# Vigilans/GomokuAI

Hardware: AMD Instinct MI355X
Metric: board-evals/s (higher is better)
Workload: dtype int32; 1 GPU; batched AC-automaton position eval (K1), 65536 random-opening boards per GPU, 15x15, inputs resident in HBM; boards_per_gpu=65536, parallelism=boards sharded by rank, no collective, launch=hipGraph replay of the K steps

## Files before the change

gomokuai_amd/csrc/eval_kernel.hip:

```cpp
#include <algorithm>
#include <cstdlib>
#include <vector>

#include "capi_common.h"
#include "host_staging.h"

namespace {

constexpr int kBoardsPerBlock = 16;
constexpr int kGroupBoards = 16;
constexpr int kThreads = 64 * kBoardsPerBlock;
constexpr int kCells = 225;
constexpr int kQueueCap = 448;
constexpr int kMaxBlocksPerCu = 1;
constexpr int kBurstEvery = 12;
static_assert(kBurstEvery >= 1 && kBurstEvery <= kGroupBoards, "every burst of a run needs a board of the run to go with");
[[maybe_unused]] constexpr int kTimelineSlots = 8;

constexpr int kScoreWords = 4 * kCells;
constexpr int kCntWords = 3 * kCells + 1;
constexpr int kZeroWords = kScoreWords + kCntWords;
constexpr int kLineWords = 96;
constexpr int kColBase = 20, kDiagBase = 36, kAntiBase = 65;
#ifndef GMK_K1_TOTALS_COPIES
#define GMK_K1_TOTALS_COPIES 8
#endif
constexpr int kTotalsCopies = GMK_K1_TOTALS_COPIES;
constexpr int kMiscWords = 48;
constexpr int kBoardWords = kZeroWords + kLineWords + kQueueCap + kMiscWords;
static_assert(kZeroWords % 4 == 0 && kBoardWords % 4 == 0, "16-byte alignment of the per-board blocks");
constexpr int kPrefixTableWords = gmk::kPrefixWords;
constexpr int kStaticTableWords = kLineWords + 512 + 1560 + 2 * kPrefixTableWords + 4;

constexpr int kLaneRecordVecs = 2;
constexpr int kSegPads = 2;
constexpr int kScanSteps = 17;
constexpr int kScanPrefixSyms = 4;
constexpr int kPairedLanes = 8, kFirstPairedLane = 64 - kPairedLanes;
constexpr int kSeamStepLong = 8 + kSegPads, kSeamStepShort = 7 + kSegPads;

__device__ __forceinline__ int dir_stride(int dir) { return (0x0E100F01u >> (8 * dir)) & 0xFFu; }

__device__ __forceinline__ uint64_t line_symbols(uint32_t line_word, int len) {
    return static_cast<uint64_t>(line_word) | (0xAull << (2 * len));
}

__device__ __forceinline__ const __attribute__((address_space(3))) uint32_t* lds_word(uint32_t byte_address) {
    return reinterpret_cast<const __attribute__((address_space(3))) uint32_t*>(static_cast<uintptr_t>(byte_address));
}

__device__ __forceinline__ const __attribute__((address_space(3))) uint16_t* lds_half(uint32_t byte_address) {
    return reinterpret_cast<const __attribute__((address_space(3))) uint16_t*>(static_cast<uintptr_t>(byte_address));
}

__device__ __forceinline__ __attribute__((address_space(3))) uint32_t* lds_word_rw(uint32_t byte_address) {
    return reinterpret_cast<__attribute__((address_space(3))) uint32_t*>(static_cast<uintptr_t>(byte_address));
}

__device__ __forceinline__ uint32_t dfa_address(uint32_t table_word, uint32_t four) {
    uint32_t addr;
    asm("v_bfi_b32 %0, %1, %2, %3" : "=v"(addr) : "s"(0x3FF3u), "v"(table_word), "v"(four));
    return addr;
}

__device__ __forceinline__ uint32_t place_advance(uint32_t place, uint32_t lines_word) {
    uint32_t next;
    asm("v_add_u32_sdwa %0, %1, %2 dst_sel:DWORD dst_unused:UNUSED_PAD src0_sel:DWORD src1_sel:BYTE_3" : "=v"(next) : "v"(place), "v"(lines_word));
    return next;
}

template <int kFirstLane>
__device__ __forceinline__ uint32_t place_jump(uint32_t place, int jump) {
    static_assert(kFirstLane >= 0 && kFirstLane < 64 && kFirstLane % 4 == 0, "four lanes of one DPP bank");
    constexpr int kRow = kFirstLane / 16, kBank = (kFirstLane % 16) / 4;
    asm("s_nop 1\n\tv_add_u32_dpp %0, %1, %0 quad_perm:[0,1,2,3] row_mask:%2 bank_mask:%3" : "+v"(place) : "v"(jump), "n"(1 << kRow), "n"(1 << kBank));
    return place;
}

__device__ __forceinline__ uint32_t queue_entry(uint32_t table_word, uint32_t place) {
    uint32_t entry;
    asm("v_bfi_b32 %0, %1, %2, %3" : "=v"(entry) : "s"(0x1FFFFu), "v"(place), "v"(table_word));
    return entry;
}

typedef unsigned short v2u16 __attribute__((ext_vector_type(2)));
__device__ __forceinline__ uint32_t pk_dec_u16(uint32_t word) {
    const v2u16 ones = {1, 1};
    return __builtin_bit_cast(uint32_t, static_cast<v2u16>(__builtin_bit_cast(v2u16, word) - ones));
}

__device__ __forceinline__ void store_saddr(uint32_t byte_offset, int32_t value, unsigned long long base) {
    asm volatile("global_store_dword %0, %1, %2" : : "v"(byte_offset), "v"(value), "s"(base) : "memory");
}

template <int kImm, bool kNt>
__device__ __forceinline__ void store_saddr_imm(uint32_t byte_offset, int32_t value, unsigned long long base) {
    static_assert(kImm >= 0 && kImm < 4096, "the immediate offset of a global store has 13 bits, signed");
    if (kNt) asm volatile("global_store_dword %0, %1, %2 offset:%3 nt" : : "v"(byte_offset), "v"(value), "s"(base), "n"(kImm) : "memory");
    else asm volatile("global_store_dword %0, %1, %2 offset:%3" : : "v"(byte_offset), "v"(value), "s"(base), "n"(kImm) : "memory");
}

__device__ __forceinline__ void wave_phase_fence() {
    __builtin_amdgcn_fence(__ATOMIC_RELEASE, "wavefront");
    __builtin_amdgcn_wave_barrier();
    __builtin_amdgcn_fence(__ATOMIC_ACQUIRE, "wavefront");
}

__device__ __forceinline__ void deposit_match(uint32_t w0, uint32_t w1, int cell_at, int dir, int back_step,
                                              uint32_t* s_scores, uint32_t* s_cnt, uint32_t* s_misc, uint32_t* totals ) {
    const int type = w0 & 15, fav = (w0 >> 4) & 1;
    if (type == 8) { atomicOr(&s_misc[1], fav ? 1u : 2u); return; }
    atomicAdd(&totals[type], fav ? 0x10000u : 1u);
    const int endcell = cell_at + static_cast<int>((w0 >> 27) & 1u) * back_step;
    const uint32_t score = dir >= 2 ? (w1 >> 16) : (w1 & 0xFFFFu);
    unsigned long long* pair = reinterpret_cast<unsigned long long*>(s_scores) + fav;
    const uint32_t lo_opp = fav ? score : 0u, hi_opp = fav ? 0u : score;
    const uint32_t tslot = 5u - static_cast<uint32_t>(type);
    const bool feeds = tslot < 3u;
    uint32_t* cnt = s_cnt + (feeds ? tslot : 0u) * kCells;
    const uint32_t one = 1u << (4 * (fav * 4 + dir));
    const int n_dep = (w0 >> 8) & 7;
#pragma unroll
    for (int d = 0; d < 4; ++d) {
        if (d >= n_dep) break;
        const uint32_t f = (w0 >> (11 + 4 * d)) & 15u;
        const int c = endcell + static_cast<int>(f & 7u) * back_step;
        const bool both = (f & 8u) != 0u;
        atomicAdd(&pair[2 * c], (static_cast<unsigned long long>(both ? score : hi_opp) << 32) | (both ? score : lo_opp));
        if (both && feeds) atomicAdd(&cnt[c], one);
    }
}

__device__ __forceinline__ int counter_match(uint32_t w0, int k, int want) {
    const int type = w0 & 15, len = (w0 >> 5) & 7;
    const int back = k - static_cast<int>((w0 >> 27) & 1u) - 6;
    if (!w0 || type != want || back < 0 || back >= len) return -1;
    const int n_dep = (w0 >> 8) & 7;
    bool on_q = false;
#pragma unroll
    for (int d = 0; d < 4; ++d) {
        const uint32_t f = (w0 >> (11 + 4 * d)) & 15u;
        on_q |= d < n_dep && f == (8u | static_cast<uint32_t>(back));
    }
    return on_q ? back : -1;
}

__device__ __forceinline__ void add_counter_cells(uint32_t w0, int back, int q, int stride, uint32_t* opp) {
    const int n_dep = (w0 >> 8) & 7, endcell = q + back * stride;
#pragma unroll
    for (int d = 0; d < 4; ++d) {
        const uint32_t f = (w0 >> (11 + 4 * d)) & 15u;
        if (d < n_dep && static_cast<int>(f & 7u) != back) atomicAdd(&opp[4 * (endcell - static_cast<int>(f & 7u) * stride)], 600u);
    }
}

[[maybe_unused]] constexpr int kDensTiles = 7;
__host__ __device__ constexpr int dens_kt_lo(int m) { return (((32 * m) / 15 - 3) < 0 ? 0 : (32 * m) / 15 - 3) / 2; }
__host__ __device__ constexpr int dens_kt_hi(int m) { return (((32 * m + 31) / 15 + 3) > 14 ? 14 : (32 * m + 31) / 15 + 3) / 2; }
constexpr int kWtabDy = 13, kWtabEntryWords = 4, kWtabKindWords = kWtabDy * 15 * kWtabEntryWords, kWtabWords = 2 * kWtabKindWords;
__host__ __device__ constexpr int block_weight(int dy, int dx) {
    constexpr int w[4][7] = {{1, 3, 4, 0, 4, 3, 1}, {0, 3, 5, 4, 5, 3, 0}, {0, 4, 3, 3, 3, 4, 0}, {2, 0, 0, 1, 0, 0, 2}};
    return w[dy < 0 ? -dy : dy][dx + 3];
}

typedef int v4i __attribute__((ext_vector_type(4)));
typedef int v16i __attribute__((ext_vector_type(16)));

template <bool kFull, int KIND, int M>
__device__ __forceinline__ void density_tile_pass(const uint32_t (&own_rows)[8], int n_live, int lane,
                                                  const v4i* __restrict__ s_wtab, const uint4* __restrict__ s_occ, int32_t* __restrict__ group_out,
                                                  unsigned long long& board_base , const uint2* __restrict__ s_lut, int plane_stride) {
    constexpr int lo = dens_kt_lo(M), hi = dens_kt_hi(M), nk = hi - lo + 1;
    const int n = lane & 31, h = lane >> 5;
    const uint4 occ_lo = s_occ[4 * M + 2 * h], occ_hi = s_occ[4 * M + 2 * h + 1];
    const uint32_t occ[8] = {occ_lo.x, occ_lo.y, occ_lo.z, occ_lo.w, occ_hi.x, occ_hi.y, occ_hi.z, occ_hi.w};
    const int cell = 32 * M + n, yo = (cell * 0x8889) >> 19, xo = cell - 15 * yo;
    const v4i* w = s_wtab + KIND * (kWtabKindWords / kWtabEntryWords) + (2 * lo + h - yo + 6) * 15 + xo;
    v16i acc = {0, 0, 0, 0, 0, 0, 0, 0, 0, 0, 0, 0, 0, 0, 0, 0};
#pragma unroll
    for (int k = 0; k < nk; ++k) {
        const uint32_t r = (own_rows[lo + k] >> (16 * h)) & 0x7FFFu;
        const uint2 b0 = s_lut[r & 255u], b1 = s_lut[r >> 8];
        const v4i stones = {static_cast<int>(b0.x), static_cast<int>(b0.y), static_cast<int>(b1.x), static_cast<int>(b1.y)};
        acc = __builtin_amdgcn_mfma_i32_32x32x32_i8(stones, w[30 * k], acc, 0, 0, 0);
    }
    const uint32_t at = static_cast<uint32_t>(KIND * plane_stride + 32 * M + n + h * (2 * 4 * plane_stride));
    if (kFull) {
        const uint32_t at_white = 4u * at, at_black = 4u * (at + 2u * static_cast<uint32_t>(plane_stride));
#pragma unroll
        for (int i = 0; i < 16; i += 2) {
            const int neg = __builtin_amdgcn_sbfe(static_cast<int>(occ[i / 2]), n, 1);
            store_saddr(at_black, acc[i] ^ neg, board_base);
            store_saddr(at_white, acc[i + 1] ^ neg, board_base);
            board_base += static_cast<long long>(i == 14 ? -13 : i % 4 ? 3 : 1) * (4 * 4 * plane_stride);
            asm volatile("" : "+s"(board_base));
        }
    } else {
        int32_t* out = group_out + at;
#pragma unroll
        for (int i = 0; i < 16; i += 2) {
            const int b = 4 * (i / 4) + (i % 4) / 2;
            const int neg = __builtin_amdgcn_sbfe(static_cast<int>(occ[i / 2]), n, 1);
            asm volatile("" : "+s"(n_live));
            if (b + 2 * h < n_live && plane_stride > 0) {
                out[b * 4 * plane_stride + 1 * 2 * plane_stride] = acc[i] ^ neg;
                out[b * 4 * plane_stride + 0 * 2 * plane_stride] = acc[i + 1] ^ neg;
            }
        }
    }
}

template <bool kFull>
__device__ __forceinline__ void density_planes_out(const uint16_t* __restrict__ planes, int n_boards, int first_board, int lane,
                                                   const v4i* __restrict__ s_wtab, uint32_t* __restrict__ s_occ, int32_t* __restrict__ out_density,
                                                   const uint2* __restrict__ s_lut, int plane_stride) {
    const int n = lane & 31, plane = n & 1, board = first_board + (n >> 1);
    uint32_t own[8], other[8];
    {
        const uint4* p = reinterpret_cast<const uint4*>(planes + static_cast<size_t>(kFull || board < n_boards ? board : first_board) * 32);
        const uint4 a0 = p[plane * 2], a1 = p[plane * 2 + 1], b0 = p[2 - plane * 2], b1 = p[3 - plane * 2];
        own[0] = a0.x; own[1] = a0.y; own[2] = a0.z; own[3] = a0.w; own[4] = a1.x; own[5] = a1.y; own[6] = a1.z; own[7] = a1.w;
        other[0] = b0.x; other[1] = b0.y; other[2] = b0.z; other[3] = b0.w; other[4] = b1.x; other[5] = b1.y; other[6] = b1.z; other[7] = b1.w;
    }
    if ((lane & 33) == 0) {
        const int bg = lane >> 1;
        uint32_t* slot = s_occ + 8 * ((bg >> 1) & 1) + 2 * (bg >> 2) + (bg & 1);
#pragma unroll
        for (int m = 0; m < kDensTiles; ++m) {
            const int y0 = (32 * m) / 15, y1 = (32 * m + 31) / 15;
            uint32_t occ = 0;
#pragma unroll
            for (int y = y0; y <= y1; ++y) {
                const uint32_t both = own[y / 2] | other[y / 2];
                const uint32_t r = ((y & 1) ? both >> 16 : both) & 0x7FFFu;
                const int at = 15 * y - 32 * m;
                occ |= at >= 0 ? r << at : r >> -at;
            }
            slot[16 * m] = occ;
        }
    }
    if ((lane >> 5) == 0 && (kFull || (board < n_boards && plane_stride > 0))) {
        uint32_t c224 = 0, w224 = 0;
#pragma unroll
        for (int dy = -3; dy <= 0; ++dy) {
            const int y = 14 + dy;
            const uint32_t r = (y & 1) ? own[y >> 1] >> 16 : own[y >> 1] & 0xFFFFu;
#pragma unroll
            for (int dx = -3; dx <= 0; ++dx) {
                if (block_weight(dy, dx) == 0) continue;
                const uint32_t bit = (r >> (14 + dx)) & 1u;
                c224 += bit;
                w224 += bit * static_cast<uint32_t>(block_weight(dy, dx));
            }
        }
        const uint32_t neg = 0u - (((own[7] | other[7]) >> 14) & 1u);
        int32_t* out = out_density + static_cast<size_t>(board) * 4 * plane_stride + (1 - plane) * 2 * plane_stride;
        out[224] = static_cast<int32_t>(c224 ^ neg);
        out[plane_stride + 224] = static_cast<int32_t>(w224 ^ neg);
    }
    const int n_live = __builtin_amdgcn_readfirstlane(n_boards - first_board);
    int32_t* group_out = out_density + static_cast<size_t>(first_board) * 4 * plane_stride;
    const uint4* occ_words = reinterpret_cast<const uint4*>(s_occ);
    const unsigned long long group_bits = reinterpret_cast<unsigned long long>(group_out);
    unsigned long long board_base = static_cast<unsigned long long>(static_cast<uint32_t>(__builtin_amdgcn_readfirstlane(static_cast<int>(group_bits >> 32)))) << 32
                                    | static_cast<uint32_t>(__builtin_amdgcn_readfirstlane(static_cast<int>(group_bits)));
    asm volatile("" : "+s"(board_base));
#define GMK_PASS(K, M) density_tile_pass<kFull, K, M>(own, n_live, lane, s_wtab, occ_words, group_out, board_base, s_lut, plane_stride); __builtin_amdgcn_sched_barrier(0);
    GMK_PASS(0, 0) GMK_PASS(1, 0) GMK_PASS(0, 1) GMK_PASS(1, 1) GMK_PASS(0, 2) GMK_PASS(1, 2) GMK_PASS(0, 3) GMK_PASS(1, 3)
    GMK_PASS(0, 4) GMK_PASS(1, 4) GMK_PASS(0, 5) GMK_PASS(1, 5) GMK_PASS(0, 6) GMK_PASS(1, 6)
#undef GMK_PASS
}

__global__ __launch_bounds__(kThreads)
void eval_positions_kernel(const uint16_t* __restrict__ planes, int n_boards, int groups_each, int groups_extra,
                           int32_t* __restrict__ out_scores, int32_t* __restrict__ out_density,
                           uint32_t* __restrict__ out_totals, int32_t* __restrict__ out_status,
                           const uint4* __restrict__ g_stage, int stage_vecs, int trans_words, int record_words,
                           int phase_mask_arg, unsigned long long* __restrict__ prof, unsigned long long* __restrict__ timeline) {
#ifdef GMK_PROFILE
    unsigned long long* const tl_row = timeline ? timeline + (static_cast<size_t>(blockIdx.x) * kBoardsPerBlock + (threadIdx.x >> 6)) * kTimelineSlots : nullptr;
#define GMK_TL(slot, value) do { if (tl_row && (threadIdx.x & 63) == 0) tl_row[slot] = (value); } while (0)
    GMK_TL(0, __builtin_amdgcn_s_memtime());
    unsigned long long tl_last_board = 0, tl_burst_clocks = 0;
    int tl_bursts = 0;
    const int phase_mask = phase_mask_arg;
    unsigned long long t_acc[12] = {0, 0, 0, 0, 0, 0, 0, 0, 0, 0, 0, 0}, t_prev = __builtin_amdgcn_s_memtime();
#define GMK_STAMP(k) do { if (prof) { const unsigned long long t_now_ = __builtin_amdgcn_s_memtime(); t_acc[k] += t_now_ - t_prev; t_prev = t_now_; } } while (0)
#else
    constexpr int phase_mask = 0x7F;
    (void)phase_mask_arg; (void)prof; (void)timeline;
#define GMK_TL(slot, value) do { } while (0)
#ifdef GMK_K1_MARKERS
#define GMK_STAMP(k) asm volatile("; gmk_mark " #k)
#else
#define GMK_STAMP(k) do { } while (0)
#endif
#endif
    extern __shared__ __attribute__((aligned(16))) uint32_t lds[];
    const uint4* s_rec = reinterpret_cast<const uint4*>(lds + trans_words);
    uint32_t* s_static = lds + trans_words + record_words;

    const int tid = threadIdx.x;
    const uint4 stage_a = g_stage[min(tid, stage_vecs - 1)], stage_b = g_stage[min(tid + kThreads, stage_vecs - 1)];
    const uint4* lane_record = g_stage + stage_vecs + kLaneRecordVecs * (tid & 63);
    const uint4 lane_lines = lane_record[0], lane_consts = lane_record[1];
    uint32_t* s_pads = s_static;
    uint2* s_lut = reinterpret_cast<uint2*>(s_static + kLineWords);
    uint32_t* s_wtab_words = s_static + kLineWords + 512;
    const v4i* s_wtab = reinterpret_cast<const v4i*>(s_wtab_words);
    const uint32_t scan_prefix_at = static_cast<uint32_t>(trans_words + record_words + kLineWords + 512 + kWtabWords) * 4u;
    const uint32_t root_prefix_at = scan_prefix_at + 4u * kPrefixTableWords;
    uint32_t* s_handout = s_wtab_words + kWtabWords + 2 * kPrefixTableWords;

    const int wave = __builtin_amdgcn_readfirstlane(threadIdx.x >> 6), lane0 = threadIdx.x & 63;
    uint32_t* s_scores = lds + trans_words + record_words + kStaticTableWords + wave * kBoardWords;
    uint32_t* s_cnt = s_scores + kScoreWords;
    uint32_t* s_lines = s_scores + kZeroWords;
    uint32_t* s_queue = s_lines + kLineWords;
    uint32_t* s_misc = s_queue + kQueueCap;
#ifndef GMK_K1_TOTALS_HOT
    uint32_t* const my_totals = s_queue + kQueueCap - 8 * kTotalsCopies + (lane0 & (kTotalsCopies - 1)) * 8;
#else
    uint32_t* const my_totals = s_misc + 4;
#endif

    GMK_STAMP(0);

    const bool planes_out = out_density != nullptr && (phase_mask & 64) && !(phase_mask & 1024);
    int lane = lane0;
    const uint32_t lines_word = lane_lines.x, place_word = lane_lines.y;
    const uint32_t line_init_lo = lane_lines.z, line_init_hi = lane_lines.w;
    const uint32_t cell_row4 = lane_consts.x, cell_col = lane_consts.y, norm_a = lane_consts.z, norm_b = lane_consts.w;
    uint32_t* s_rows = s_misc + 16;
    const uint16_t* row_ptr = planes + (lane & 15);
    uint32_t next_black = 0, next_white = 0, cur_black = 0, cur_white = 0;
    auto fetch_row = [&](int b) {
        const uint16_t* p = row_ptr + static_cast<size_t>(min(b, n_boards - 1)) * 32;
        next_black = p[0];
        next_white = p[16];
    };
    auto take_row = [&](int lane_m, int b) -> uint32_t { return lane_m < 16 && b < n_boards ? cur_black | (cur_white << 16) : 0u; };

    const int wg_block = static_cast<int>(blockIdx.x);
    const int wg_g0 = groups_each * wg_block + min(wg_block, groups_extra);
    const int wg_groups = groups_each + (wg_block < groups_extra ? 1 : 0);
    const int wg_first = wg_g0 * kGroupBoards, wg_boards = min(wg_groups * kGroupBoards, n_boards - wg_first);
    auto hand_out = [&]() -> int {
        uint32_t v = 0;
        if (lane0 == 0) v = atomicAdd(s_handout, 1u);
        return __builtin_amdgcn_readfirstlane(static_cast<int>(v));
    };
    int idx = wave, boards_done = 0;
    if (idx < wg_boards) fetch_row(wg_first + idx);
    {
        uint4* s_stage = reinterpret_cast<uint4*>(lds);
        if (tid < stage_vecs) s_stage[tid] = stage_a;
        if (tid + kThreads < stage_vecs) s_stage[tid + kThreads] = stage_b;
        for (int i = tid + 2 * kThreads; i < stage_vecs; i += kThreads) s_stage[i] = g_stage[i];
    }
    asm volatile("" : "+v"(next_black), "+v"(next_white));
    GMK_TL(1, __builtin_amdgcn_s_memtime());
#pragma unroll 1
    for (;;) {
#ifdef GMK_K1_MARKERS
        GMK_STAMP(10);
#endif
        const bool live = idx < wg_boards;
        const int board = wg_first + idx;
        cur_black = next_black; cur_white = next_white;
        int idx_next = idx;
        if (live) { idx_next = boards_done == 0 ? kBoardsPerBlock + wave : hand_out(); fetch_row(wg_first + min(idx_next, wg_boards - 1)); }
        GMK_STAMP(11);

        uint32_t late_row = 0;
        int late_lane = lane, late_gate = 0, late_gw = 0;
        auto late_piece = [&](int piece) {
            if (piece == 0) {
#ifndef GMK_K1_TOTALS_HOT
                if (lane < 8 * kTotalsCopies) s_queue[kQueueCap - 8 * kTotalsCopies + lane] = 0;
#endif
            } else if (piece <= 3) {
                constexpr int kVecs = kCntWords / 4;
                static_assert(kVecs > 128 && kVecs <= 192, "three pieces of 64 lanes clear the counters");
                const int i = 64 * (piece - 1);
                if (i + 64 <= kVecs || late_lane < kVecs - i) (reinterpret_cast<uint4*>(s_cnt) + lane)[i] = make_uint4(0u, 0u, 0u, 0u);
            } else if (piece == 4) {
                uint32_t cnt = static_cast<uint32_t>(__popc(late_row & 0x7FFFu)) | (static_cast<uint32_t>(__popc(late_row >> 16)) << 16);
                cnt += static_cast<uint32_t>(__builtin_amdgcn_update_dpp(0, static_cast<int>(cnt), 0x118, 0xF, 0xF, false));
                cnt += static_cast<uint32_t>(__builtin_amdgcn_update_dpp(0, static_cast<int>(cnt), 0x114, 0xF, 0xF, false));
                cnt += static_cast<uint32_t>(__builtin_amdgcn_update_dpp(0, static_cast<int>(cnt), 0x112, 0xF, 0xF, false));
                cnt += static_cast<uint32_t>(__builtin_amdgcn_update_dpp(0, static_cast<int>(cnt), 0x111, 0xF, 0xF, false));
                if (late_lane == 15) s_misc[0] = cnt;
            } else if (piece == 5) {
                const uint32_t r = late_row;
                const v2u16 rr = __builtin_bit_cast(v2u16, r);
                const uint32_t l1 = __builtin_bit_cast(uint32_t, static_cast<v2u16>(rr << 1)), l2 = __builtin_bit_cast(uint32_t, static_cast<v2u16>(rr << 2)), l3 = __builtin_bit_cast(uint32_t, static_cast<v2u16>(rr << 3));
                const uint32_t r1 = __builtin_bit_cast(uint32_t, static_cast<v2u16>(rr >> 1)), r2 = __builtin_bit_cast(uint32_t, static_cast<v2u16>(rr >> 2)), r3 = __builtin_bit_cast(uint32_t, static_cast<v2u16>(rr >> 3));
                const int far = static_cast<int>(r | l3 | r3), near = static_cast<int>(r | l1 | l2 | r1 | r2);
                uint32_t g = l1 | l2 | l3 | r1 | r2 | r3;
                g |= static_cast<uint32_t>(__builtin_amdgcn_update_dpp(0, near, 0x111, 0xF, 0xF, true)) | static_cast<uint32_t>(__builtin_amdgcn_update_dpp(0, near, 0x101, 0xF, 0xF, true));
                g |= static_cast<uint32_t>(__builtin_amdgcn_update_dpp(0, near, 0x112, 0xF, 0xF, true)) | static_cast<uint32_t>(__builtin_amdgcn_update_dpp(0, near, 0x102, 0xF, 0xF, true));
                g |= static_cast<uint32_t>(__builtin_amdgcn_update_dpp(0, far, 0x113, 0xF, 0xF, true)) | static_cast<uint32_t>(__builtin_amdgcn_update_dpp(0, far, 0x103, 0xF, 0xF, true));
                const uint32_t empty = ~(r | (r >> 16)) & 0x7FFFu;
                if (lane < 15) s_rows[3 + lane] = r;
                late_gate = static_cast<int>(g & (empty | (empty << 16)));
                late_gw = __builtin_amdgcn_ds_bpermute(static_cast<int>(cell_row4 & 0xFFu), late_gate);
            } else if (piece <= 9) {
                const int pass = piece - 6;
                const uint32_t gw = static_cast<uint32_t>(late_gw) >> ((cell_col >> (8 * pass)) & 0xFFu);
                static_assert(4 * 256 - kScoreWords <= kCntWords, "the fourth write's lanes behind the last cell land on counter words");
                reinterpret_cast<uint4*>(s_scores)[64 * pass + lane] = make_uint4(static_cast<uint32_t>(__builtin_amdgcn_sbfe(static_cast<int>(gw), 16, 1)) & 160u, 0u, 0u,
                                                                                  static_cast<uint32_t>(__builtin_amdgcn_sbfe(static_cast<int>(gw), 0, 1)) & 160u);
                if (pass < 3) late_gw = __builtin_amdgcn_ds_bpermute(static_cast<int>((cell_row4 >> (8 * (pass + 1))) & 0xFFu), late_gate);
            }
        };
        constexpr int kLatePieces = 10;
        static_assert(kLatePieces <= kScanSteps - kScanPrefixSyms + 1, "a piece per lookup");
        if (live) {
            int lane_m = lane;
            asm volatile("" : "+v"(lane_m));
            s_lines[lane] = line_init_lo;
            if (lane_m < kLineWords - 64) s_lines[64 + lane] = line_init_hi;
            if (lane_m < kMiscWords) s_misc[lane] = 0;
            const uint32_t my_row = take_row(lane_m, board);
            late_row = my_row; late_lane = lane_m;
            wave_phase_fence();
            {
                const int y = lane >> 2, part = lane & 3;
                const uint32_t row = __shfl(my_row, min(y, 14));
                uint32_t row_sym = 0;
                uint32_t y2 = 2u * static_cast<uint32_t>(y), y4 = 4u * static_cast<uint32_t>(y);
                asm volatile("" : "+v"(y2), "+v"(y4));
                for (uint32_t m = lane < 60 ? (row | (row >> 16)) & (0xFu << (4 * part)) & 0x7FFFu : 0u; m; m &= m - 1u) {
                    const int x = __ffs(m) - 1;
                    const uint32_t code = ((row >> x) & 1u) | 2u;
                    const uint32_t at_x = code << (2 * x), at_y = code << y2;
                    row_sym |= at_x;
                    char* const col = reinterpret_cast<char*>(s_lines + x);
                    atomicXor(reinterpret_cast<uint32_t*>(col) + kColBase, at_y);
                    atomicXor(reinterpret_cast<uint32_t*>(col - y4) + (kDiagBase + 14), at_x);
                    atomicXor(reinterpret_cast<uint32_t*>(col + y4) + kAntiBase, at_y);
                }
                if (row_sym) atomicXor(&s_lines[y], row_sym);
            }
            wave_phase_fence();
            GMK_STAMP(1);
        }
#ifdef GMK_PROFILE
        if (boards_done == 0) GMK_TL(2, __builtin_amdgcn_s_memtime());
#endif
        if (boards_done == 0) __syncthreads();
#ifdef GMK_PROFILE
        if (boards_done == 0) GMK_TL(3, __builtin_amdgcn_s_memtime());
        if (live) { tl_bursts = 0; tl_burst_clocks = 0; }
#endif
        if (live) {
            int n_queued = 0;
            if (phase_mask & 2) {
                const int len_a = static_cast<int>(lines_word & 31u) - kSegPads, len_b = static_cast<int>((lines_word >> 5) & 31u) - kSegPads;
                uint64_t syms = line_symbols(s_lines[(lines_word >> 10) & 127u] >> norm_a, len_a);
                syms |= line_symbols(s_lines[(lines_word >> 17) & 127u] >> norm_b, len_b) << (2 * (len_a + kSegPads));
                syms |= 0xAAAAAAAAAAAAAAAAull << (2 * (len_a + len_b + 2 * kSegPads));
                const uint32_t cur = static_cast<uint32_t>(syms) << 2;
                const uint32_t rest = static_cast<uint32_t>(syms >> 28);
                const uint32_t q_base = static_cast<uint32_t>(s_queue - lds) * 4u;
                constexpr int kQueueFlagAt = kQueueCap - 64;
                const uint32_t q_full = q_base + 4u * kQueueFlagAt;
                static_assert(kQueueFlagAt > 0 && (kQueueFlagAt - 1) + 64 < kQueueCap, "the deposits' read one round ahead stays inside the queue");
                uint32_t q_at = q_base;
                uint32_t pend_at = 0, pend_entry = 0;
                bool pend = false;
                auto flush = [&]() { if (pend) *lds_word_rw(pend_at) = pend_entry; };
                uint32_t place = place_word;
                const int seam_jump = __builtin_amdgcn_sbfe(static_cast<int>(place_word), 17, 10);
                auto push = [&](uint32_t word, int step) {
                    const bool emits = word > 0x1FFFFu;
                    const unsigned long long emitters = __ballot(emits);
                    const uint32_t ahead = __builtin_amdgcn_mbcnt_hi(static_cast<uint32_t>(emitters >> 32), __builtin_amdgcn_mbcnt_lo(static_cast<uint32_t>(emitters), 0u));
                    pend = emits;
                    pend_at = q_at + 4u * ahead;
                    if (step > kScanPrefixSyms) place = place_advance(place, lines_word);
                    static_assert(kPairedLanes == 8, "two banks of four lanes: the long first lines in front");
                    if (step == kSeamStepShort) place = place_jump<kFirstPairedLane + 4>(place, seam_jump);
                    if (step == kSeamStepLong) place = place_jump<kFirstPairedLane>(place, seam_jump);
                    pend_entry = queue_entry(word, place);
                    asm volatile("" : "+v"(pend_at), "+v"(pend_entry));
                    q_at = min(q_at + 4u * static_cast<uint32_t>(__popcll(emitters)), q_full);
                };
                uint32_t tw = *lds_half(scan_prefix_at + __builtin_amdgcn_ubfe(cur, 1, 9));
                __builtin_amdgcn_sched_barrier(0);
                late_piece(0);
                __builtin_amdgcn_sched_barrier(0);
#pragma unroll
                for (int step = kScanPrefixSyms; step < kScanSteps; ++step) {
                    const int nth = step - kScanPrefixSyms + 1;
                    const uint32_t four = step < 15 ? __builtin_amdgcn_ubfe(cur, 2 * step, 4) : __builtin_amdgcn_ubfe(rest, 2 * (step - 15), 4);
                    const uint32_t addr = dfa_address(tw, four);
                    const uint32_t before = tw;
                    tw = *lds_word(addr);
                    flush();
                    __builtin_amdgcn_sched_barrier(0);
                    if (step > kScanPrefixSyms) push(before, step - 1);
                    if (nth < kLatePieces) { late_piece(nth); __builtin_amdgcn_sched_barrier(0); }
                }
                flush();
                push(tw, kScanSteps - 1);
                flush();
                n_queued = static_cast<int>((q_at - q_base) >> 2);
                if (q_at >= q_full) s_misc[2] = 1;
            }
#ifdef GMK_PROFILE
            else {
#pragma unroll
                for (int piece = 0; piece < kLatePieces; ++piece) late_piece(piece);
            }
#endif
            wave_phase_fence();
            GMK_STAMP(2);

            if (phase_mask & 4) {
                uint32_t qe_next = s_queue[lane];
                for (int m = lane; m < n_queued; m += 64) {
                    const uint32_t qe = qe_next;
                    qe_next = s_queue[m + 64];
                    const uint4 rec_now = s_rec[qe >> 17];
                    const int cell_at = qe & 511u, dir = (qe >> 9) & 3u;
                    const int back_step = __builtin_amdgcn_sbfe(static_cast<int>(qe), 11, 6);
                    deposit_match(rec_now.x, rec_now.y, cell_at, dir, back_step, s_scores, s_cnt, s_misc, my_totals);
                    if (rec_now.z) deposit_match(rec_now.z, rec_now.w, cell_at, dir, back_step, s_scores, s_cnt, s_misc, my_totals);
                }
            }
            wave_phase_fence();
#ifndef GMK_K1_TOTALS_HOT
            if (lane < 8) {
                const uint32_t* t = s_queue + kQueueCap - 8 * kTotalsCopies + lane;
                uint32_t sum = 0;
#pragma unroll
                for (int c = 0; c < kTotalsCopies; ++c) sum += t[8 * c];
                s_misc[4 + lane] = sum;
            }
#endif
            GMK_STAMP(3);

            int n_cand = 0;
            if (phase_mask & 8) {
                uint32_t any_cnt[4];
    #pragma unroll
                for (int pass = 0; pass < 4; ++pass) {
                    const int qc = min(64 * pass + lane, kCells - 1);
                    any_cnt[pass] = s_cnt[qc] | s_cnt[kCells + qc] | s_cnt[2 * kCells + qc];
                }
    #pragma unroll
                for (int pass = 0; pass < 4; ++pass) {
                    const int q = 64 * pass + lane;
                    const uint32_t any = any_cnt[pass];
                    const uint32_t hot = any & (pk_dec_u16(any) | 0xEEEEEEEEu);
                    const unsigned long long pushers = __ballot(hot != 0u) & (pass < 3 ? ~0ull : (1ull << (kCells - 192)) - 1ull);
                    if (pushers) {
                        if (hot != 0u && (pass < 3 || lane < kCells - 192)) {
                            const int slot = n_cand + static_cast<int>(__builtin_amdgcn_mbcnt_hi(static_cast<uint32_t>(pushers >> 32),
                                                                       __builtin_amdgcn_mbcnt_lo(static_cast<uint32_t>(pushers), 0u)));
                            if (slot < kQueueCap / 2) s_queue[slot] = static_cast<uint32_t>(q) | ((hot & 0xFFFFu) ? 0x100u : 0u) | ((hot >> 16) ? 0x200u : 0u);
                        }
                        n_cand += __popcll(pushers);
                    }
                }
            }
            wave_phase_fence();
            GMK_STAMP(4);

            if (n_cand > kQueueCap / 2) { s_misc[2] = 1; n_cand = kQueueCap / 2; }
            if (phase_mask & 2048) n_cand = 0;
            constexpr int kRescanFlush = kQueueCap / 2 - 2 * 64;
            static_assert(kRescanFlush > 0 && kRescanFlush + 2 * 64 <= kQueueCap / 2, "a round of phase 3b fits behind the flush level");
            int n_comp_q = 0;
            if (phase_mask & 8)
            for (int v0 = 0; v0 < 2 * n_cand; v0 += 64) {
                const int v = v0 + lane;
                const int flag_shift = 8 + (v & 1);
                const uint32_t ce = s_queue[v >> 1];
                const int q = ce & 255, c = v & 1;
                bool queue = false;
                uint32_t ent1 = 0, ent2 = 0;
                if (v < 2 * n_cand && ((ce >> flag_shift) & 1u)) {
                    const uint32_t f3 = (s_cnt[q] >> (16 * c)) & 0xFFFFu, fd = (s_cnt[kCells + q] >> (16 * c)) & 0xFFFFu, f2 = (s_cnt[2 * kCells + q] >> (16 * c)) & 0xFFFFu;
                    uint32_t dens = 0;
                    const int qy = (q * 0x8889) >> 19, qx = q - 15 * qy;
                    {
                        const int half = c ? 0 : 16;
    #pragma unroll
                        for (int dy = -3; dy <= 3; ++dy) {
                            const uint32_t pattern = dy == 0 ? 0x77u : (dy == 3 || dy == -3) ? 0x49u : 0x3Eu;
                            const uint32_t mask = ((pattern << qx) >> 3) & 0x7FFFu;
                            dens += __popc((s_rows[3 + qy + dy] >> half) & mask);
                        }
                    }
                    if (dens >= 2u) {
                        const uint32_t up3 = (f3 >> 1) | (f3 >> 2) | (f3 >> 3), upd = (fd >> 1) | (fd >> 2) | (fd >> 3), up2 = (f2 >> 1) | (f2 >> 2) | (f2 >> 3);
                        const uint32_t sel3 = (f3 | up3) & 0x1111u;
                        const uint32_t seld = (fd | upd) & 0x1111u & ~sel3;
                        const uint32_t sel2 = (f2 | up2) & 0x1111u & ~(sel3 | seld);
                        const uint32_t strong = sel3 | seld, any_dir = strong | sel2;
                        const uint32_t twice_strong = (sel3 & up3) | (seld & upd), twice = twice_strong | (sel2 & up2);
                        const int n_comp = __popc(any_dir) + __popc(twice), threes = __popc(strong) + __popc(twice_strong);
                        if (n_comp < 2) {
                            s_misc[2] = 1;
                        } else {
                            const int ctype = min(threes, 2);
                            atomicAdd(&s_misc[12 + ctype], c ? 0x10000u : 1u);
                            const uint32_t crit = 600u * static_cast<uint32_t>(n_comp);
                            atomicAdd(reinterpret_cast<unsigned long long*>(s_scores) + 2 * q + c, (static_cast<unsigned long long>(crit) << 32) | crit);
                            queue = n_comp < 3 && !sel3;
                            const uint32_t b1 = static_cast<uint32_t>(__ffs(any_dir) - 1);
                            const uint32_t others = any_dir & (any_dir - 1u);
                            const uint32_t b2 = others ? static_cast<uint32_t>(__ffs(others) - 1) : b1;
                            const uint32_t ux = static_cast<uint32_t>(qx), uy = static_cast<uint32_t>(qy);
                            const uint32_t lines = (static_cast<uint32_t>(kColBase) << 8 | static_cast<uint32_t>(kDiagBase + 14) << 16 | static_cast<uint32_t>(kAntiBase) << 24)
                                                   + ((ux << 8) * 0x10101u) + uy * 0xFF0001u;
                            const uint32_t slots = ux * 0x0101u + uy * 0x1010u;
                            const uint32_t head = static_cast<uint32_t>(q) | (static_cast<uint32_t>(c) << 8);
                            auto entry = [&](uint32_t b) {
                                const uint32_t tslot = ((seld >> b) & 1u) ? 1u : 2u;
                                return head | (b >> 2) << 9 | tslot << 11 | __builtin_amdgcn_ubfe(lines, 2 * b, 8) << 13 | __builtin_amdgcn_ubfe(slots, b, 4) << 20;
                            };
                            ent1 = entry(b1);
                            ent2 = entry(b2);
                        }
                    }
                }
                const unsigned long long queuers = __ballot(queue);
                if (queue) {
                    const uint32_t slot = static_cast<uint32_t>(n_comp_q) + 2u * __builtin_amdgcn_mbcnt_hi(static_cast<uint32_t>(queuers >> 32),
                                                                                                          __builtin_amdgcn_mbcnt_lo(static_cast<uint32_t>(queuers), 0u));
                    s_queue[kQueueCap / 2 + slot] = ent1;
                    s_queue[kQueueCap / 2 + slot + 1] = ent2;
                }
                n_comp_q += 2 * __popcll(queuers);
                if (v0 + 64 < 2 * n_cand && n_comp_q <= kRescanFlush) continue;
            wave_phase_fence();
            GMK_STAMP(5);

            if (phase_mask & 16) {
                const int n_comp = n_comp_q;
                int lane_4 = lane;
                asm volatile("" : "+v"(lane_4));
                const int grp = lane_4 / 7, kk = lane_4 - 7 * grp, k = 6 + kk, start = k > 7 ? k - 7 : 0;
                for (int m0 = 0; m0 < n_comp; m0 += 9) {
                    const int m = m0 + grp;
                    const bool on = lane < 63 && m < n_comp;
                    const uint32_t ent = on ? s_queue[kQueueCap / 2 + m] : 0u;
                    const int q = ent & 255, c = (ent >> 8) & 1, dir = (ent >> 9) & 3, tslot = (ent >> 11) & 3;
                    const int stride = dir_stride(dir);
                    uint32_t hit_w0 = 0;
                    int hit_back = -1;
                    if (on) {
                        const uint32_t line = (ent >> 13) & 127u;
                        const uint32_t word = s_lines[line] | s_pads[line];
                        const int first = static_cast<int>((ent >> 20) & 15u) + start - 6;
                        const uint32_t cur = __builtin_amdgcn_alignbit(first >= 0 ? 0xAAAAAAAAu : word, first >= 0 ? word : 0xAAAAAAAAu,
                                                                       static_cast<uint32_t>(2 * first) & 31u) << 2;
                        uint32_t tw = *lds_half(root_prefix_at + __builtin_amdgcn_ubfe(cur, 1, 9)), tw_third = 0;
    #pragma unroll
                        for (int i = 4; i < 8; ++i) {
                            if (i == 7) tw_third = tw;
                            tw = *lds_word(dfa_address(tw, __builtin_amdgcn_ubfe(cur, 2 * i, 4)));
                        }
                        if (kk == 0) tw = tw_third;
                        if ((gmk::dev_trans_kinds(tw) >> tslot) & 1u) {
                            const uint4 rec = s_rec[gmk::dev_trans_record(tw)];
                            const int want = 5 - tslot;
                            hit_back = counter_match(rec.x, k, want);
                            hit_w0 = rec.x;
                            if (hit_back < 0) { hit_back = counter_match(rec.z, k, want); hit_w0 = rec.z; }
                        }
                    }
                    const unsigned long long hits = __ballot(hit_back >= 0);
                    const uint32_t mine = static_cast<uint32_t>(hits >> (7 * grp)) & 0x7Fu;
                    if (hit_back >= 0 && (mine & ((1u << kk) - 1u)) == 0u) add_counter_cells(hit_w0, hit_back, q, stride, s_scores + (c ? 2 : 1));
                }
            }
            n_comp_q = 0;
            wave_phase_fence();
            GMK_STAMP(6);
            }

        }

        asm volatile("" : "+v"(next_black), "+v"(next_white));
        GMK_STAMP(7);

        if (!live) break;
        const int burst = idx / kBurstEvery;
        if (planes_out && burst * kBurstEvery == idx && burst < wg_groups) {
#ifdef GMK_PROFILE
            const unsigned long long tl_burst_from = __builtin_amdgcn_s_memtime();
#endif
            int lane_p = lane0, first_p = (wg_g0 + burst) * kGroupBoards;
            asm volatile("" : "+v"(lane_p), "+s"(first_p));
            const int plane_stride = (phase_mask & 512) ? 0 : (phase_mask & 256) ? 256 : kCells;
            if (first_p + kGroupBoards <= n_boards && plane_stride > 0) density_planes_out<true>(planes, n_boards, first_p, lane_p, s_wtab, s_queue, out_density, s_lut, plane_stride);
            else density_planes_out<false>(planes, n_boards, first_p, lane_p, s_wtab, s_queue, out_density, s_lut, plane_stride);
            GMK_STAMP(8);
#ifdef GMK_PROFILE
            ++tl_bursts; tl_burst_clocks += __builtin_amdgcn_s_memtime() - tl_burst_from;
#endif
        }
#ifdef GMK_K1_MARKERS
        GMK_STAMP(12);
#endif
        if (live && (phase_mask & 32)) {
            int lane_b = lane;
            asm volatile("" : "+v"(lane_b));
            const uint32_t lane_off = 4u * static_cast<uint32_t>(lane_b);
            if (out_scores) {
                const unsigned long long dst = reinterpret_cast<unsigned long long>(out_scores + static_cast<size_t>(board) * kScoreWords);
                const int4* src = reinterpret_cast<const int4*>(s_scores);
                const int4 v0 = src[lane_b], v1 = src[lane_b + 64], v2 = src[lane_b + 128], v3 = src[min(lane_b + 192, kCells - 1)];
#ifdef GMK_K1_PLAIN_SCORES
                constexpr bool kNt = false;
#else
                constexpr bool kNt = true;
#endif
#define GMK_STORE(words, v) store_saddr_imm<4 * (words), kNt>(lane_off, v, dst)
                const bool tail = lane_b + 192 < kCells;
                GMK_STORE(0, v0.x); GMK_STORE(64, v1.x); GMK_STORE(128, v2.x); if (tail) GMK_STORE(192, v3.x);
                GMK_STORE(kCells, v0.y); GMK_STORE(kCells + 64, v1.y); GMK_STORE(kCells + 128, v2.y); if (tail) GMK_STORE(kCells + 192, v3.y);
                GMK_STORE(2 * kCells, v0.z); GMK_STORE(2 * kCells + 64, v1.z); GMK_STORE(2 * kCells + 128, v2.z); if (tail) GMK_STORE(2 * kCells + 192, v3.z);
                GMK_STORE(3 * kCells, v0.w); GMK_STORE(3 * kCells + 64, v1.w); GMK_STORE(3 * kCells + 128, v2.w); if (tail) GMK_STORE(3 * kCells + 192, v3.w);
#undef GMK_STORE
            }
            if (out_totals) {
                const unsigned long long dst = reinterpret_cast<unsigned long long>(out_totals + static_cast<size_t>(board) * 11);
                if (lane_b < 11) store_saddr_imm<0, false>(lane_off, static_cast<int32_t>(s_misc[4 + lane_b]), dst);
            }
            if (out_status) {
                const uint32_t stones = static_cast<uint32_t>(__builtin_amdgcn_readfirstlane(static_cast<int>(s_misc[0])));
                const uint32_t wbits = static_cast<uint32_t>(__builtin_amdgcn_readfirstlane(static_cast<int>(s_misc[1])));
                const uint32_t flagged = static_cast<uint32_t>(__builtin_amdgcn_readfirstlane(static_cast<int>(s_misc[2])));
                const int stones_b = stones & 0xFFFFu, stones_w = stones >> 16;
                const int winner = (wbits & 1u) ? 1 : (wbits & 2u) ? -1 : 0;
                const bool over = winner != 0 || stones_b + stones_w == kCells;
                const int to_move = over ? 0 : (stones_b == stones_w ? 1 : -1);
                const int word = (over ? 1 : 0) | ((flagged || phase_mask != 0x7F) ? 2 : 0) | ((winner & 0xFF) << 8) | ((to_move & 0xFF) << 16);
                const unsigned long long dst = reinterpret_cast<unsigned long long>(out_status + board);
                if (lane_b == 0) store_saddr_imm<0, false>(lane_off, word, dst);
            }
        }
        wave_phase_fence();
        GMK_STAMP(9);
#ifdef GMK_PROFILE
        tl_last_board = __builtin_amdgcn_s_memtime();
#endif
        idx = idx_next; ++boards_done;
    }
#ifdef GMK_PROFILE
    GMK_TL(4, tl_last_board);
    GMK_TL(6, static_cast<unsigned long long>(tl_bursts) | static_cast<unsigned long long>(boards_done) << 16);
    GMK_TL(7, tl_burst_clocks);
    GMK_TL(5, __builtin_amdgcn_s_memtime());
    if (prof && lane0 == 0) {
        for (int k = 0; k < 12; ++k) atomicAdd(&prof[k], t_acc[k]);
        atomicAdd(&prof[15], 1ull);
    }
#endif
#undef GMK_STAMP
#undef GMK_TL
}

struct LineJob { int len, x0, y0, dir; };

int lane_tables(uint32_t* pads_out, uint32_t* records_out) {
    std::vector<LineJob> lines;
    for (int i = 0; i < 15; ++i) lines.push_back({15, 0, i, 0});
    for (int i = 0; i < 15; ++i) lines.push_back({15, i, 0, 1});
    for (int d = -10; d <= 10; ++d) lines.push_back({15 - std::abs(d), d > 0 ? d : 0, d > 0 ? 0 : -d, 2});
    for (int k = 4; k <= 24; ++k) { const int x0 = std::min(k, 14); lines.push_back({std::min(k, 28 - k) + 1, x0, k - x0, 3}); }
    std::stable_sort(lines.begin(), lines.end(), [](const LineJob& a, const LineJob& b) { return a.len > b.len; });
    if (lines.size() != 64 + kPairedLanes) { gmk::set_error("lane lines: %zu lines for 64 lanes and %d second lines", lines.size(), kPairedLanes); return GMK_ERR_STATE; }
    auto line_word = [](const LineJob& l) { return l.dir == 0 ? l.y0 : l.dir == 1 ? kColBase + l.x0 : l.dir == 2 ? kDiagBase + l.x0 - l.y0 + 14 : kAntiBase + l.x0 + l.y0; };
    auto stride_of = [](int dir) { return dir == 0 ? 1 : dir == 1 ? 15 : dir == 2 ? 16 : 14; };
    auto first_cell = [](const LineJob& l) { return l.y0 * 15 + l.x0; };
    auto second_line = [](int lane) { return lane < kFirstPairedLane ? -1 : lane < kFirstPairedLane + 4 ? lane + 12 : lane + 4; };
    uint32_t lines_words[64], place_words[64];
    int steps = 0;
    for (int lane = 0; lane < 64; ++lane) {
        const LineJob& a = lines[lane];
        const LineJob* b = second_line(lane) < 0 ? nullptr : &lines[second_line(lane)];
        if (a.len < kScanPrefixSyms) { gmk::set_error("lane lines: lane %d starts with a line of %d cells, the scan's prefix read takes %d", lane, a.len, kScanPrefixSyms); return GMK_ERR_STATE; }
        if (b && b->dir != a.dir) { gmk::set_error("lane lines: lane %d walks lines of directions %d and %d", lane, a.dir, b->dir); return GMK_ERR_STATE; }
        const int seg_a = a.len + kSegPads, seg_b = b ? b->len + kSegPads : kSegPads, stride = stride_of(a.dir);
        if (b && seg_a != (lane < kFirstPairedLane + 4 ? kSeamStepLong : kSeamStepShort)) { gmk::set_error("lane lines: lane %d steps to its second line at step %d", lane, seg_a); return GMK_ERR_STATE; }
        const int jump = b ? first_cell(*b) - (first_cell(a) + seg_a * stride) : 0;
        if (jump < -512 || jump > 511) { gmk::set_error("lane lines: lane %d jumps %d cells", lane, jump); return GMK_ERR_STATE; }
        lines_words[lane] = static_cast<uint32_t>(seg_a | seg_b << 5 | line_word(a) << 10 | (b ? line_word(*b) : 15) << 17 | stride << 24);
        place_words[lane] = static_cast<uint32_t>(first_cell(a) + kScanPrefixSyms * stride) | static_cast<uint32_t>(a.dir) << 9 | (static_cast<uint32_t>(-stride) & 63u) << 11
                            | (static_cast<uint32_t>(jump) & 1023u) << 17;
        steps = std::max(steps, seg_a + (b ? seg_b : 0));
        uint32_t place = place_words[lane];
        const int jump_field = static_cast<int>(place_words[lane] << 5) >> 22;
        for (int step = kScanPrefixSyms; step < kScanSteps; ++step) {
            if (step > kScanPrefixSyms) place += lines_words[lane] >> 24;
            if (step == kSeamStepShort && lane >= kFirstPairedLane + 4) place += static_cast<uint32_t>(jump_field);
            if (step == kSeamStepLong && lane >= kFirstPairedLane && lane < kFirstPairedLane + 4) place += static_cast<uint32_t>(jump_field);
            const bool second = b && step >= seg_a;
            const LineJob& l = second ? *b : a;
            const int cell = first_cell(l) + (step - (second ? seg_a : 0)) * stride_of(l.dir);
            const uint32_t want = static_cast<uint32_t>(cell) | static_cast<uint32_t>(l.dir) << 9 | (static_cast<uint32_t>(-stride_of(l.dir)) & 63u) << 11;
            if (cell < 0 || cell > 511 || (place & 0x1FFFFu) != want) {
                gmk::set_error("lane lines: lane %d step %d carries place 0x%05x, the plain statement gives 0x%05x", lane, step, place & 0x1FFFFu, want);
                return GMK_ERR_STATE;
            }
        }
    }
    uint32_t init[kLineWords] = {};
    for (int i = 0; i < 15; ++i) init[i] = init[kColBase + i] = 0x3FFFFFFFu;
    for (int d = 0; d <= 28; ++d) init[kDiagBase + d] = init[kAntiBase + d] = ((1u << (2 * (15 - std::abs(d - 14)))) - 1u) << (2 * std::max(0, d - 14));
    uint32_t consts[64][4];
    for (int lane = 0; lane < 64; ++lane) {
        uint32_t row4 = 0, col = 0;
        for (int pass = 0; pass < 4; ++pass) {
            const int c = std::min(64 * pass + lane, kCells - 1);
            if (64 * pass + lane >= kCells) { row4 |= static_cast<uint32_t>(4 * 16) << (8 * pass); continue; }
            row4 |= static_cast<uint32_t>(4 * (c / 15)) << (8 * pass);
            col |= static_cast<uint32_t>(c % 15) << (8 * pass);
        }
        consts[lane][0] = row4;
        consts[lane][1] = col;
        for (int k = 0; k < 2; ++k) {
            const int at = k == 0 ? lane : second_line(lane);
            consts[lane][2 + k] = at < 0 ? 0u : lines[at].dir == 2 ? 2u * static_cast<uint32_t>(lines[at].x0) : lines[at].dir == 3 ? 2u * static_cast<uint32_t>(lines[at].y0) : 0u;
        }
    }
    for (int i = 0; i < kLineWords; ++i) pads_out[i] = ~init[i] & 0xAAAAAAAAu;
    for (int lane = 0; lane < 64; ++lane) {
        uint32_t* r = records_out + 8 * lane;
        r[0] = lines_words[lane]; r[1] = place_words[lane];
        r[2] = init[lane]; r[3] = init[std::min(64 + lane, kLineWords - 1)];
        for (int k = 0; k < 4; ++k) r[4 + k] = consts[lane][k];
    }
    if (steps != kScanSteps) { gmk::set_error("lane lines: %d scan steps, the kernel is built for %d", steps, kScanSteps); return GMK_ERR_STATE; }
    return GMK_OK;
}

int density_weights(int8_t* t ) {
    for (int kind = 0; kind < 2; ++kind)
        for (int dy = -3; dy <= 3; ++dy)
            for (int xo = 0; xo < 15; ++xo)
                for (int j = 0; j < 15; ++j) {
                    if (std::abs(j - xo) > 3) continue;
                    const int w = block_weight(dy, j - xo);
                    t[((static_cast<size_t>(kind) * kWtabDy + dy + 6) * 15 + xo) * 16 + j] = static_cast<int8_t>(kind == 0 ? (w != 0) : w);
                }
    for (int cell = 0; cell < 224; ++cell)
        for (int kt = dens_kt_lo(cell / 32); kt <= dens_kt_hi(cell / 32); ++kt)
            for (int h = 0; h < 2; ++h) {
                const int dy = 2 * kt + h - cell / 15;
                if (dy < -6 || dy > 6) { gmk::set_error("density weight table: dy %d of cell %d out of range", dy, cell); return GMK_ERR_STATE; }
            }
    for (int cell = 0; cell < 224; ++cell)
        for (int dy = -3; dy <= 3; ++dy) {
            const int y = cell / 15 + dy, m = cell / 32;
            if (y < 0 || y > 14) continue;
            if (y / 2 < dens_kt_lo(m) || y / 2 > dens_kt_hi(m)) { gmk::set_error("density weight table: row %d of cell %d is not covered", y, cell); return GMK_ERR_STATE; }
        }
    return GMK_OK;
}

int scan_start_row(const gmk::DeviceTables& t, uint32_t* row_out) {
    constexpr uint32_t kPad = 2;
    const std::vector<uint32_t>& tr = t.dev_trans;
    const uint32_t n = static_cast<uint32_t>(t.n_states);
    if (n == 0 || tr.size() != static_cast<size_t>(n) * 4) { gmk::set_error("K1 scan: no automaton"); return GMK_ERR_STATE; }
    const uint32_t first = tr[kPad], start = gmk::dev_trans_row(first);
    if (gmk::dev_trans_record(first) != 0 || start % 16 != 0 || start / 16 >= n) { gmk::set_error("K1 scan: the root emits on '?' or leaves the table"); return GMK_ERR_STATE; }
    const uint32_t loop = tr[start / 4 + kPad];
    if (gmk::dev_trans_record(loop) != 0 || gmk::dev_trans_row(loop) != start) { gmk::set_error("K1 scan: state %u does not loop on '?' without emitting", start / 16); return GMK_ERR_STATE; }
    for (uint32_t s = 0; s < n; ++s) {
        const uint32_t mid = gmk::dev_trans_row(tr[s * 4 + kPad]);
        if (mid % 16 != 0 || mid / 16 >= n || gmk::dev_trans_row(tr[mid / 4 + kPad]) != start) { gmk::set_error("K1 scan: \"??\" from state %u does not lead to state %u", s, start / 16); return GMK_ERR_STATE; }
    }
    *row_out = start;
    return GMK_OK;
}

int scan_prefix_table(const gmk::DeviceTables& t, uint32_t start, uint16_t* out ) {
    const std::vector<uint32_t>& tr = t.dev_trans;
    for (uint32_t key = 0; key < 256; ++key) {
        uint32_t row = start;
        bool cells = true, reports = false;
        for (int i = 0; i < kScanPrefixSyms; ++i) {
            const uint32_t sym = (key >> (2 * i)) & 3u;
            if (row % 16 != 0 || row / 4 + sym >= tr.size()) { gmk::set_error("K1 scan prefix: a walk from state %u leaves the table", start / 16); return GMK_ERR_STATE; }
            const uint32_t tw = tr[row / 4 + sym];
            cells = cells && sym != 2u;
            reports = reports || gmk::dev_trans_record(tw) != 0;
            row = gmk::dev_trans_row(tw);
        }
        if (cells && reports) { gmk::set_error("K1 scan prefix: the cells of key 0x%02x report a match within four symbols of state %u", key, start / 16); return GMK_ERR_STATE; }
        out[key] = static_cast<uint16_t>(row);
    }
    return GMK_OK;
}

int build_stage_image(const gmk::DeviceState& st, uint4** d_out, int* stage_vecs) {
    const size_t trans_words = static_cast<size_t>(st.n_states) * 4, record_words = static_cast<size_t>(st.n_records) * 4;
    std::vector<uint32_t> rest(kStaticTableWords + 64 * 4 * kLaneRecordVecs, 0u);
    uint32_t* pads = rest.data(), *lut = pads + kLineWords, *wtab = lut + 512, *scan_prefix = wtab + kWtabWords, *root_prefix = scan_prefix + kPrefixTableWords,
              *handout = root_prefix + kPrefixTableWords, *records = handout + 4;
    int rc = lane_tables(pads, records);
    if (rc != GMK_OK) return rc;
    for (uint32_t b = 0; b < 256; ++b) { lut[2 * b] = ((b & 15u) * 0x204081u) & 0x01010101u; lut[2 * b + 1] = ((b >> 4) * 0x204081u) & 0x01010101u; }
    rc = density_weights(reinterpret_cast<int8_t*>(wtab));
    if (rc != GMK_OK) return rc;
    handout[0] = 2u * kBoardsPerBlock;
    const gmk::DeviceTables& tables = gmk::production_automaton().device();
    rc = scan_start_row(tables, &handout[1]);
    if (rc != GMK_OK) return rc;
    uint16_t halves[256];
    rc = scan_prefix_table(tables, handout[1], halves);
    if (rc != GMK_OK) return rc;
    if (tables.dev_prefix4.size() != 256) { gmk::set_error("K1 tables: no four-symbol prefix table of the root"); return GMK_ERR_STATE; }
    for (int i = 0; i < kPrefixTableWords; ++i) {
        scan_prefix[i] = static_cast<uint32_t>(halves[2 * i]) | static_cast<uint32_t>(halves[2 * i + 1]) << 16;
        root_prefix[i] = static_cast<uint32_t>(tables.dev_prefix4[2 * i]) | static_cast<uint32_t>(tables.dev_prefix4[2 * i + 1]) << 16;
    }
    const size_t staged_words = trans_words + record_words + kStaticTableWords;
    if (staged_words % 4 != 0) { gmk::set_error("K1 tables: %zu staged words are not whole 16-byte pieces", staged_words); return GMK_ERR_STATE; }
    uint32_t* d = nullptr;
    GMK_HIP_CHECK(hipMalloc(&d, (trans_words + record_words + rest.size()) * sizeof(uint32_t)));
    GMK_HIP_CHECK(hipMemcpy(d, st.d_trans, trans_words * sizeof(uint32_t), hipMemcpyDeviceToDevice));
    GMK_HIP_CHECK(hipMemcpy(d + trans_words, st.d_records, record_words * sizeof(uint32_t), hipMemcpyDeviceToDevice));
    GMK_HIP_CHECK(hipMemcpy(d + trans_words + record_words, rest.data(), rest.size() * sizeof(uint32_t), hipMemcpyHostToDevice));
    *d_out = reinterpret_cast<uint4*>(d);
    *stage_vecs = static_cast<int>(staged_words / 4);
    return GMK_OK;
}

struct Launch { int grid, n_groups, groups_each, groups_extra; size_t lds; };

Launch plan_launch(int n, const gmk::DeviceState& st) {
    Launch l;
// ... 113 lines not shown
```

Measured before the change: 650.1 million board-evals/s.

## Split phase-3b candidate work across four lanes and drop density gate

Phase 3b now maps each candidate/color pair onto a quad of four lanes instead of one lane per pair. Lanes 0 and 1 of a quad each build one of the two queue entries, and lane 0 alone does the score atomics. The density popcount filter (dens >= 2) is removed, so every flagged candidate proceeds to classification, which may change results or add work. counter_match also replaces its per-dependency loop with a SWAR nibble-equality test. Only 16 pairs per round instead of 64 means more loop iterations and ballots per candidate list.

```diff
diff --git a/gomokuai_amd/csrc/eval_kernel.hip b/gomokuai_amd/csrc/eval_kernel.hip
--- a/gomokuai_amd/csrc/eval_kernel.hip
+++ b/gomokuai_amd/csrc/eval_kernel.hip
@@ -136,12 +136,8 @@
     const int back = k - static_cast<int>((w0 >> 27) & 1u) - 6;
     if (!w0 || type != want || back < 0 || back >= len) return -1;
     const int n_dep = (w0 >> 8) & 7;
-    bool on_q = false;
-#pragma unroll
-    for (int d = 0; d < 4; ++d) {
-        const uint32_t f = (w0 >> (11 + 4 * d)) & 15u;
-        on_q |= d < n_dep && f == (8u | static_cast<uint32_t>(back));
-    }
+    const uint32_t x = ((w0 >> 11) & 0xFFFFu) ^ (static_cast<uint32_t>(back) * 0x1111u + 0x8888u);
+    const bool on_q = ((x - 0x1111u) & ~x & 0x8888u & ((1u << (4 * n_dep)) - 1u)) != 0u;
     return on_q ? back : -1;
 }
 
@@ -571,31 +567,24 @@
 
             if (n_cand > kQueueCap / 2) { s_misc[2] = 1; n_cand = kQueueCap / 2; }
             if (phase_mask & 2048) n_cand = 0;
-            constexpr int kRescanFlush = kQueueCap / 2 - 2 * 64;
-            static_assert(kRescanFlush > 0 && kRescanFlush + 2 * 64 <= kQueueCap / 2, "a round of phase 3b fits behind the flush level");
+            constexpr int kPairsPerRound = 16;
+            constexpr int kRescanFlush = kQueueCap / 2 - 2 * kPairsPerRound;
+            static_assert(kRescanFlush > 0 && kRescanFlush + 2 * kPairsPerRound <= kQueueCap / 2, "a round of phase 3b fits behind the flush level");
             int n_comp_q = 0;
             if (phase_mask & 8)
-            for (int v0 = 0; v0 < 2 * n_cand; v0 += 64) {
-                const int v = v0 + lane;
+            for (int v0 = 0; v0 < 2 * n_cand; v0 += kPairsPerRound) {
+                int lane_3 = lane;
+                asm volatile("" : "+v"(lane_3));
+                const int j = lane_3 & 3, v = v0 + (lane_3 >> 2);
                 const int flag_shift = 8 + (v & 1);
                 const uint32_t ce = s_queue[v >> 1];
                 const int q = ce & 255, c = v & 1;
                 bool queue = false;
-                uint32_t ent1 = 0, ent2 = 0;
+                uint32_t ent = 0;
                 if (v < 2 * n_cand && ((ce >> flag_shift) & 1u)) {
                     const uint32_t f3 = (s_cnt[q] >> (16 * c)) & 0xFFFFu, fd = (s_cnt[kCells + q] >> (16 * c)) & 0xFFFFu, f2 = (s_cnt[2 * kCells + q] >> (16 * c)) & 0xFFFFu;
-                    uint32_t dens = 0;
                     const int qy = (q * 0x8889) >> 19, qx = q - 15 * qy;
                     {
-                        const int half = c ? 0 : 16;
-    #pragma unroll
-                        for (int dy = -3; dy <= 3; ++dy) {
-                            const uint32_t pattern = dy == 0 ? 0x77u : (dy == 3 || dy == -3) ? 0x49u : 0x3Eu;
-                            const uint32_t mask = ((pattern << qx) >> 3) & 0x7FFFu;
-                            dens += __popc((s_rows[3 + qy + dy] >> half) & mask);
-                        }
-                    }
-                    if (dens >= 2u) {
                         const uint32_t up3 = (f3 >> 1) | (f3 >> 2) | (f3 >> 3), upd = (fd >> 1) | (fd >> 2) | (fd >> 3), up2 = (f2 >> 1) | (f2 >> 2) | (f2 >> 3);
                         const uint32_t sel3 = (f3 | up3) & 0x1111u;
                         const uint32_t seld = (fd | upd) & 0x1111u & ~sel3;
@@ -604,39 +593,36 @@
                         const uint32_t twice_strong = (sel3 & up3) | (seld & upd), twice = twice_strong | (sel2 & up2);
                         const int n_comp = __popc(any_dir) + __popc(twice), threes = __popc(strong) + __popc(twice_strong);
                         if (n_comp < 2) {
-                            s_misc[2] = 1;
+                            if (j == 0) s_misc[2] = 1;
                         } else {
-                            const int ctype = min(threes, 2);
-                            atomicAdd(&s_misc[12 + ctype], c ? 0x10000u : 1u);
-                            const uint32_t crit = 600u * static_cast<uint32_t>(n_comp);
-                            atomicAdd(reinterpret_cast<unsigned long long*>(s_scores) + 2 * q + c, (static_cast<unsigned long long>(crit) << 32) | crit);
+                            if (j == 0) {
+                                const int ctype = min(threes, 2);
+                                atomicAdd(&s_misc[12 + ctype], c ? 0x10000u : 1u);
+                                const uint32_t crit = 600u * static_cast<uint32_t>(n_comp);
+                                atomicAdd(reinterpret_cast<unsigned long long*>(s_scores) + 2 * q + c, (static_cast<unsigned long long>(crit) << 32) | crit);
+                            }
                             queue = n_comp < 3 && !sel3;
-                            const uint32_t b1 = static_cast<uint32_t>(__ffs(any_dir) - 1);
                             const uint32_t others = any_dir & (any_dir - 1u);
-                            const uint32_t b2 = others ? static_cast<uint32_t>(__ffs(others) - 1) : b1;
+                            const uint32_t pick = (j == 0 || !others) ? any_dir : others;
+                            const uint32_t b = static_cast<uint32_t>(__ffs(pick) - 1);
                             const uint32_t ux = static_cast<uint32_t>(qx), uy = static_cast<uint32_t>(qy);
                             const uint32_t lines = (static_cast<uint32_t>(kColBase) << 8 | static_cast<uint32_t>(kDiagBase + 14) << 16 | static_cast<uint32_t>(kAntiBase) << 24)
                                                    + ((ux << 8) * 0x10101u) + uy * 0xFF0001u;
                             const uint32_t slots = ux * 0x0101u + uy * 0x1010u;
-                            const uint32_t head = static_cast<uint32_t>(q) | (static_cast<uint32_t>(c) << 8);
-                            auto entry = [&](uint32_t b) {
-                                const uint32_t tslot = ((seld >> b) & 1u) ? 1u : 2u;
-                                return head | (b >> 2) << 9 | tslot << 11 | __builtin_amdgcn_ubfe(lines, 2 * b, 8) << 13 | __builtin_amdgcn_ubfe(slots, b, 4) << 20;
-                            };
-                            ent1 = entry(b1);
-                            ent2 = entry(b2);
+                            const uint32_t tslot = ((seld >> b) & 1u) ? 1u : 2u;
+                            ent = static_cast<uint32_t>(q) | (static_cast<uint32_t>(c) << 8) | (b >> 2) << 9 | tslot << 11 | __builtin_amdgcn_ubfe(lines, 2 * b, 8) << 13
+                                  | __builtin_amdgcn_ubfe(slots, b, 4) << 20;
                         }
                     }
                 }
-                const unsigned long long queuers = __ballot(queue);
-                if (queue) {
+                const unsigned long long queuers = __ballot(queue) & 0x8888888888888888ull;
+                if (queue && j < 2) {
                     const uint32_t slot = static_cast<uint32_t>(n_comp_q) + 2u * __builtin_amdgcn_mbcnt_hi(static_cast<uint32_t>(queuers >> 32),
                                                                                                           __builtin_amdgcn_mbcnt_lo(static_cast<uint32_t>(queuers), 0u));
-                    s_queue[kQueueCap / 2 + slot] = ent1;
-                    s_queue[kQueueCap / 2 + slot + 1] = ent2;
+                    s_queue[kQueueCap / 2 + slot + static_cast<uint32_t>(j)] = ent;
                 }
                 n_comp_q += 2 * __popcll(queuers);
-                if (v0 + 64 < 2 * n_cand && n_comp_q <= kRescanFlush) continue;
+                if (v0 + kPairsPerRound < 2 * n_cand && n_comp_q <= kRescanFlush) continue;
             wave_phase_fence();
             GMK_STAMP(5);
 
```

Result: faster. 660.7 million board-evals/s, median of 6 (+1.6%).
